# Mehran-Memon/fspann-query-system

Hardware: AMD Instinct MI355X
Metric: queries/sec @ recall@10, SIFT-1M-shaped synthetic data d=128 B=256 (higher is better)
Workload: dtype f64

## Files before the change

fspann-query-system_amd/csrc/route_lazy.hip.h:

```cpp
#pragma once
#include "route.hip.h"

namespace fspann {

constexpr uint64_t kLzEmpty = ~0ull;
constexpr int kLzThreads = 256;
constexpr int kLzEntriesMax = 1024;
constexpr int kLzCollMax = 256;
constexpr int lz_ht_size(int kEnt) { return 2 * kEnt; }
constexpr int lz_sort_max(int kEnt) { return kEnt - 128; }
constexpr size_t lz_order_bytes(int TP) {
    return static_cast<size_t>(TP + 2) * 8 + ((static_cast<size_t>(TP + 1) * 4 + 7) & ~size_t(7)) + static_cast<size_t>(TP) * 8 +
           ((static_cast<size_t>(TP) * 2 + 3) & ~size_t(3));
}
constexpr size_t lz_lds_bytes(int kEnt, int TD, int P) {
    const size_t tp = static_cast<size_t>(TD) * P, ord_gk = lz_order_bytes(TD * P), gk = static_cast<size_t>(lz_sort_max(kEnt)) * 4;
    return static_cast<size_t>(lz_ht_size(kEnt)) * 8 + tp * 16 + static_cast<size_t>(kEnt) * 4 + 4096 +
           (((ord_gk > gk ? ord_gk : gk) + 7) & ~size_t(7)) + static_cast<size_t>(TD) * 8 + static_cast<size_t>(kEnt) * 2 +
           static_cast<size_t>(lz_sort_max(kEnt)) * 2 * 2 + static_cast<size_t>(TD) * 4 +
           (kEnt != 512 ? static_cast<size_t>(TD) * 4 + tp * 4 : 0);
}
static_assert(lz_lds_bytes(512, 16, 5) == 20152 && lz_lds_bytes(512, 16, 5) + 256 <= 160 * 1024 / 8, "eight per CU at 16 x 5");
constexpr int lz_stage_u(int) { return 4; }
constexpr int lz_keep(int) { return 8; }

#ifdef FSPANN_DEBUG_STAMPS
__device__ __forceinline__ long long dbg_hw_where() {
    uint32_t hw, xcc;
    asm volatile("s_getreg_b32 %0, hwreg(HW_REG_HW_ID)" : "=s"(hw));
    asm volatile("s_getreg_b32 %0, hwreg(HW_REG_XCC_ID)" : "=s"(xcc));
    return (static_cast<long long>(xcc) << 32) | hw;
}
#endif

__device__ __forceinline__ int wave_cut1024(const int32_t* bins, int need, int lane, int* before) {
    const int4* b4 = reinterpret_cast<const int4*>(bins) + lane * 4;
    const int4 v0 = b4[0], v1 = b4[1], v2 = b4[2], v3 = b4[3];
    const int vals[16] = {v0.x, v0.y, v0.z, v0.w, v1.x, v1.y, v1.z, v1.w, v2.x, v2.y, v2.z, v2.w, v3.x, v3.y, v3.z, v3.w};
    int sum = 0;
#pragma unroll
    for (int i = 0; i < 16; i++) sum += vals[i];
    int incl = sum;
#pragma unroll
    for (int off = 1; off < 64; off <<= 1) {
        const int v = __shfl_up(incl, off);
        if (lane >= off) incl += v;
    }
    const int excl = incl - sum;
    const unsigned long long bm = __ballot((incl >= need) && (excl < need));
    if (bm == 0) {
        *before = __shfl(incl, 63) - __shfl(v3.w, 63);
        return 1023;
    }
    const int src = __ffsll(static_cast<long long>(bm)) - 1;
    int cum = excl, bb = 15;
    bool found = false;
#pragma unroll
    for (int i = 0; i < 16; i++) {
        if (!found) {
            if (cum + vals[i] >= need) { bb = i; found = true; }
            else cum += vals[i];
        }
    }
    *before = __shfl(cum, src);
    return __shfl(lane * 16 + bb, src);
}

template <int kThreads, int kEnt = kLzEntriesMax, bool kChk = true, int kTD = 0, int kP = 0, bool kList = false>
__device__ __forceinline__ void route_lazy_run(const RouteParams& prm, unsigned char* smem, const int64_t q_first, const int64_t q_stride, const int block_id) {
    int4* probe_in = prm.probe_g;
    int32_t* nprobe_in = prm.nprobe_g;
    int tid = threadIdx.x;
    constexpr int nthreads = kThreads;
    constexpr int nwv = kThreads / 64;
    int lane = tid & 63, wave = __builtin_amdgcn_readfirstlane(tid >> 6);
    const int TD = kTD > 0 ? kTD : prm.TD, P = kP > 0 ? kP : prm.P, S = (kTD > 0) ? 64 : prm.S;
    const int TP = TD * P;
    const int SP = (S + 63) >> 6;

    constexpr int kLzHtSize = lz_ht_size(kEnt), kLzEntries = kEnt, kLzSortMax = lz_sort_max(kEnt);
    constexpr int kLzStageU = lz_stage_u(kEnt), kLzKeep = lz_keep(kEnt);
    static_assert(kEnt == 512 || kEnt == 1024 || kEnt == 2048, "size classes");
    static_assert(!(kChk && kEnt == 512), "the 512-entry class has no registers for the check");
    size_t o = 0;
    uint64_t* ht = reinterpret_cast<uint64_t*>(smem + o);        o += static_cast<size_t>(kLzHtSize) * 8;
    int4* plist = reinterpret_cast<int4*>(smem + o);             o += static_cast<size_t>(TP) * 16;
    uint32_t* pre = reinterpret_cast<uint32_t*>(smem + o);       o += static_cast<size_t>(kEnt) * 4;
    int32_t* bins = reinterpret_cast<int32_t*>(smem + o);        o += 1024 * 4;
    const size_t o_ord = o;
    uint2* pkv = reinterpret_cast<uint2*>(smem + o);             o += (static_cast<size_t>(TP) + 2) * 8;
    int32_t* pcs = reinterpret_cast<int32_t*>(smem + o);         o += (static_cast<size_t>(TP) + 1) * 4;
    o = (o + 7) & ~size_t(7);
    int64_t* pbase = reinterpret_cast<int64_t*>(smem + o);       o += static_cast<size_t>(TP) * 8;
    uint16_t* ord = reinterpret_cast<uint16_t*>(smem + o);
    uint32_t* gk = reinterpret_cast<uint32_t*>(smem + o_ord);
    o = o_ord + ((max(lz_order_bytes(TP), static_cast<size_t>(kLzSortMax) * 4) + 7) & ~size_t(7));
    int64_t* ids_base = reinterpret_cast<int64_t*>(smem + o);    o += static_cast<size_t>(TD) * 8;
    uint16_t* ulist = reinterpret_cast<uint16_t*>(smem + o);     o += static_cast<size_t>(kLzEntries) * 2;
    uint16_t* rk = reinterpret_cast<uint16_t*>(smem + o);        o += static_cast<size_t>(kLzSortMax) * 2;
    uint16_t* lrank = reinterpret_cast<uint16_t*>(smem + o);     o += static_cast<size_t>(kLzSortMax) * 2;
    int32_t* nprobe_l = reinterpret_cast<int32_t*>(smem + o);    o += static_cast<size_t>(TD) * 4;
    int32_t* part0 = reinterpret_cast<int32_t*>(smem + o);       if (kEnt != 512) o += static_cast<size_t>(TD) * 4;
    int32_t* pglob = reinterpret_cast<int32_t*>(smem + o);
    int32_t* c_elem = bins;
    int32_t* c_lt = bins + kLzCollMax;
    int32_t* c_id = bins + 2 * kLzCollMax;
    int32_t* c_seq = bins + 3 * kLzCollMax;

    __shared__ int s_u, s_R, s_ncoll, s_bad, s_b, s_cnt, s_short, s_susp;
    constexpr uint32_t ht_mask = kLzHtSize - 1;
    constexpr int ht_shift = (kEnt == 2048) ? 32 - 12 : (kEnt == 1024) ? 32 - 11 : 32 - 10;
    unsigned long long lt_mask = 0;

    for (int i = tid; i < TD; i += nthreads) { ids_base[i] = prm.tables[i].ids_base; if (kChk) part0[i] = static_cast<int32_t>(prm.tables[i].part_base); }
    for (int i = tid; i < kLzHtSize; i += nthreads) ht[i] = kLzEmpty;
    if (kChk && prm.bin16) for (int i = tid; i < 1024; i += nthreads) bins[i] = 0;
    if (block_id == 0 && tid == 0) *prm.ovf_next = 0;
    __syncthreads();

    auto present = [&](int32_t id) -> bool {
        uint32_t slot = (static_cast<uint32_t>(id) * 2654435761u) >> ht_shift;
        const uint32_t stp = ((static_cast<uint32_t>(id) * 0x85EBCA6Bu) >> ht_shift) | 1u;
        for (int tries = 0; tries < kLzHtSize; tries++) {
            const uint64_t e = ht[slot];
            if (e == kLzEmpty) return false;
            if (static_cast<uint32_t>(e >> 32) == static_cast<uint32_t>(id)) return true;
            slot = (slot + stp) & ht_mask;
        }
        return false;
    };
    auto insert = [&](int32_t id, uint32_t low, uint32_t* slot_out) -> bool {
        const uint64_t mine = (static_cast<uint64_t>(static_cast<uint32_t>(id)) << 32) | low;
        uint32_t slot = (static_cast<uint32_t>(id) * 2654435761u) >> ht_shift;
        const uint32_t stp = ((static_cast<uint32_t>(id) * 0x85EBCA6Bu) >> ht_shift) | 1u;
        for (int tries = 0; tries < kLzHtSize; tries++) {
            const uint64_t old = atomicCAS(reinterpret_cast<unsigned long long*>(&ht[slot]), kLzEmpty, mine);
            if (old == kLzEmpty) { *slot_out = slot; return true; }
            if (static_cast<uint32_t>(old >> 32) == static_cast<uint32_t>(id)) {
                if (static_cast<uint32_t>(old) > low) atomicMin(reinterpret_cast<unsigned long long*>(&ht[slot]), mine);
                return false;
            }
            slot = (slot + stp) & ht_mask;
        }
        s_bad = 1;
        return false;
    };

#ifdef FSPANN_DEBUG_STAMPS
#define LZ_STAMP(i) do { if (prm.dbg && tid == 0 && qi == block_id) prm.dbg[block_id * 16 + (i)] = wall_clock64(); } while (0)
#else
#define LZ_STAMP(i) do { } while (0)
#endif
#ifdef FSPANN_LZ_STOP_AFTER
#define LZ_STOP(n) if (FSPANN_LZ_STOP_AFTER == (n) && prm.nq > 0) { __syncthreads(); if (tid == 0) prm.out_count[qi] = 0;               \
        const int used_ = min(s_u, kLzEntries); for (int i_ = tid; i_ < used_; i_ += nthreads) ht[ulist[i_]] = kLzEmpty; __syncthreads(); continue; }
#else
#define LZ_STOP(n)
#endif
#define LZ_FOR_TUPLES(RA, RB, BODY)                                                                                   \
    do {                                                                                                              \
        const int nit_ = ((RB) - (RA)) * SP;                                                                          \
        for (int it0_ = wave; it0_ < nit_; it0_ += nwv * kLzStageU) {                                                 \
            uint64_t entv_[kLzStageU];                                                                                \
            int scv_[kLzStageU];                                                                                      \
            _Pragma("unroll") for (int v_ = 0; v_ < kLzStageU; v_++) {                                                \
                const int it_ = it0_ + v_ * nwv;                                                                      \
                entv_[v_] = kLzEmpty; scv_[v_] = 0;                                                                   \
                if (it_ < nit_) {                                                                                     \
                    const int rr_ = (RA) + it_ / SP, pos_ = (it_ % SP) * 64 + lane;                                   \
                    const int pi_ = ord[rr_];                                                                         \
                    const int4 pr_ = plist[pi_];                                                                      \
                    scv_[v_] = pr_.y;                                                                                 \
                    if (pos_ < pr_.w) entv_[v_] = prm.ids_bk[pbase[pi_] + pos_];                                      \
                }                                                                                                     \
            }                                                                                                         \
            _Pragma("unroll") for (int v_ = 0; v_ < kLzStageU; v_++) {                                                \
                if (it0_ + v_ * nwv >= nit_) continue;                                                                \
                int32_t id = static_cast<int32_t>(entv_[v_] >> 32);                              \
                const uint32_t bf = static_cast<uint32_t>(entv_[v_]); (void)bf;                                       \
                const int sc = scv_[v_]; (void)sc;                                                                    \
                if (id >= 0 && prm.deleted_bits && ((prm.deleted_bits[id >> 5] >> (id & 31)) & 1u)) id = -1;  \
                BODY                                                                                                  \
            }                                                                                                         \
        }                                                                                                             \
    } while (0)
#define LZ_INSERT(COND, LOW)                                                                                          \
    do {                                                                                                              \
        bool created_ = false;                                                                                        \
        uint32_t slot_ = 0;                                                                                           \
        if (COND) created_ = insert(id, (LOW), &slot_);                                                               \
        const unsigned long long bm_ = __ballot(created_);                                                            \
        if (bm_) {                                                                                                    \
            int base_ = 0;                                                                                            \
            if (lane == 0) base_ = atomicAdd(&s_u, __popcll(bm_));                                                    \
            base_ = __shfl(base_, 0);                                                                                 \
            const int at_ = base_ + __popcll(bm_ & lt_mask);                                                          \
            if (created_ && at_ < kLzEntries) ulist[at_] = static_cast<uint16_t>(slot_);                              \
        }                                                                                                             \
    } while (0)

    const int64_t nq_eff = kList ? static_cast<int64_t>(*prm.qcount) : prm.nq;
    for (int64_t qs = q_first; qs < nq_eff; qs += q_stride) {
        const int64_t qi = kList ? static_cast<int64_t>(prm.qlist[qs]) : qs;
        LZ_STAMP(0);
        if (prm.probe_G > 0) {
            const int G = (kTD > 0) ? 16 : prm.probe_G, lgG = 31 - __clz(G), ngroups = nthreads >> lgG;
            const int grp_in_wave = lane >> lgG, gl = lane & (G - 1), grp = tid >> lgG;
            int32_t* w3 = reinterpret_cast<int32_t*>(pre) + grp * (2 * P - 1) * 3;
            for (int t0 = 0; t0 < TD; t0 += ngroups) {
                const int td = t0 + grp;
                const bool act = td < TD;
                const int tdc = act ? td : 0;
                const int Wc = (kTD > 0) ? 1 : prm.W;
#ifdef FSPANN_DEBUG_STAMPS
                long long* pst = (prm.dbg && tid == 0 && qi == block_id && t0 == 0) ? prm.dbg + (static_cast<long long>(gridDim.x) + block_id) * 16 : nullptr;
#else
                long long* pst = nullptr;
#endif
                const int np = route_probe_table<int4*, kP, (kTD > 0 ? 1 : 0)>(prm, act, prm.codes + (qi * TD + tdc) * Wc, prm.tables[tdc], G, gl, grp_in_wave,
                                                                             w3, plist + tdc * P, pst);
                if (act && gl == 0) nprobe_l[td] = np;
            }
            __syncthreads();
            for (int i = tid; i < TP; i += nthreads) {
                const int td = i / P, step = i - td * P;
                int4 e = make_int4(-1, 0x7FFF, 0, 0);
                if (step < nprobe_l[td]) e = plist[i];
                plist[i] = e;
                pbase[i] = ids_base[td] + e.z;
                if (kChk) pglob[i] = part0[td] + e.x;
                pkv[i] = make_uint2((static_cast<uint32_t>(e.y) << 16) | static_cast<uint32_t>(i), static_cast<uint32_t>(e.w));
            }
        } else {
            for (int i = tid; i < TP; i += nthreads) {
                const int td = i / P, step = i - td * P;
                int4 e = make_int4(-1, 0x7FFF, 0, 0);
                if (step < nprobe_in[qi * TD + td]) e = probe_in[qi * TP + i];
                plist[i] = e;
                pbase[i] = ids_base[td] + e.z;
                if (kChk) pglob[i] = part0[td] + e.x;
                pkv[i] = make_uint2((static_cast<uint32_t>(e.y) << 16) | static_cast<uint32_t>(i), static_cast<uint32_t>(e.w));
            }
        }
        if (tid == 0) {
            s_u = 0; s_R = TP; s_ncoll = 0; s_bad = 0; s_short = 0; s_susp = 0;
            if (TP & 1) pkv[TP] = make_uint2(0xFFFFFFFFu, 0u);
        }
        __syncthreads();
        LZ_STAMP(1);
        LZ_STOP(1)
        asm volatile("" : "+v"(tid));
        lane = tid & 63; wave = __builtin_amdgcn_readfirstlane(tid >> 6);
        lt_mask = (1ull << lane) - 1ull;
        constexpr int kChkU = 5;
        uint2 chk_v[kChkU];
        int chk_n[kChkU];
        const int chk_cps = prm.bin16_shift - 2;
        const int chk_items = (kChk && prm.bin16) ? (TP << chk_cps) : 0;
        const bool chk_once = chk_items <= nthreads * kChkU;
        auto chk_load = [&](const int it0) {
#pragma unroll
            for (int v = 0; v < kChkU; v++) {
                const int it = it0 + v * nthreads;
                chk_v[v] = make_uint2(0u, 0u); chk_n[v] = 0;
                if (it < chk_items) {
                    const int pi = it >> chk_cps, ch = it & ((1 << chk_cps) - 1);
                    const int4 pr = plist[pi];
                    const int rem = pr.w - ch * 4;
                    if (pr.x >= 0 && rem > 0) {
                        chk_v[v] = *reinterpret_cast<const uint2*>(prm.bin16 + (static_cast<int64_t>(pglob[pi]) << prm.bin16_shift) + ch * 4);
                        chk_n[v] = min(rem, 4);
                    }
                }
            }
        };
        auto chk_count = [&]() {
            bool sus = false;
#pragma unroll
            for (int v = 0; v < kChkU; v++) {
#pragma unroll
                for (int k = 0; k < 4; k++) {
                    if (k < chk_n[v]) {
                        const uint32_t b16 = ((k < 2 ? chk_v[v].x : chk_v[v].y) >> ((k & 1) * 16)) & 0xFFFFu;
                        const uint32_t sh = (b16 & 7u) * 4u;
                        const uint32_t old = atomicAdd(reinterpret_cast<uint32_t*>(bins) + ((b16 & 8191u) >> 3), 1u << sh);
                        sus = sus || (((old >> sh) & 15u) >= 8u);
                    }
                }
            }
            if (sus) s_susp = 1;
        };
        if (chk_items > 0 && chk_once) chk_load(tid);
        for (int i = tid; i < TP; i += nthreads) {
            const uint2 me = pkv[i];
            const uint32_t mk = me.x;
            int rank = 0, cum = 0;
            const uint4* kv4 = reinterpret_cast<const uint4*>(pkv);
#pragma unroll 4
            for (int j = 0; j < (TP + 1) / 2; j++) {
                const uint4 kv = kv4[j];
                const bool b0 = kv.x < mk, b1 = kv.z < mk;
                rank += b0 + b1;
                cum += (b0 ? kv.y : 0u) + (b1 ? kv.w : 0u);
            }
            ord[rank] = static_cast<uint16_t>(i);
            pcs[rank] = cum;
            if ((mk >> 16) == 0x7FFFu) atomicMin(&s_R, rank);
            if (rank == TP - 1) pcs[TP] = cum + static_cast<int>(me.y);
        }
        if (chk_items > 0) {
            if (chk_once) chk_count();
            else for (int it0 = tid; it0 < chk_items; it0 += nthreads * kChkU) { chk_load(it0); chk_count(); }
        }
        __syncthreads();
        LZ_STAMP(2);
        LZ_STOP(2)
        const int R = s_R;
        bool overflow = false;
        if (chk_items > 0 && s_susp) {
            uint32_t* mark = reinterpret_cast<uint32_t*>(ht);
            uint64_t* cl = ht + 128;
            uint64_t* cf = cl + 256;
            constexpr int kChkList = 256;
            static_assert(128 + 2 * 256 <= lz_ht_size(512), "the check's scratch fits the smallest hash table");
            for (int i = tid; i < 256; i += nthreads) mark[i] = 0u;
            for (int i = tid; i < 1024; i += nthreads) bins[i] = 0;
            __syncthreads();
            for (int it = tid; it < chk_items; it += nthreads) {
                const int pi = it >> chk_cps, ch = it & ((1 << chk_cps) - 1);
                const int4 pr = plist[pi];
                const int rem = pr.w - ch * 4;
                if (pr.x < 0 || rem <= 0) continue;
                const uint2 vv = *reinterpret_cast<const uint2*>(prm.bin16 + (static_cast<int64_t>(pglob[pi]) << prm.bin16_shift) + ch * 4);
                for (int k = 0; k < min(rem, 4); k++) {
                    const uint32_t b16 = ((k < 2 ? vv.x : vv.y) >> ((k & 1) * 16)) & 0xFFFFu, f = b16 & 8191u;
                    const uint32_t sh = (f & 7u) * 4u;
                    const uint32_t old = atomicAdd(reinterpret_cast<uint32_t*>(bins) + (f >> 3), 1u << sh);
                    if (((old >> sh) & 15u) >= 8u) atomicOr(&mark[f >> 5], 1u << (f & 31u));
                }
            }
            __syncthreads();
            for (int it = tid; it < chk_items; it += nthreads) {
                const int pi = it >> chk_cps, ch = it & ((1 << chk_cps) - 1);
                const int4 pr = plist[pi];
                const int rem = pr.w - ch * 4;
                if (pr.x < 0 || rem <= 0) continue;
                const uint2 vv = *reinterpret_cast<const uint2*>(prm.bin16 + (static_cast<int64_t>(pglob[pi]) << prm.bin16_shift) + ch * 4);
                for (int k = 0; k < min(rem, 4); k++) {
                    const uint32_t b16 = ((k < 2 ? vv.x : vv.y) >> ((k & 1) * 16)) & 0xFFFFu, f = b16 & 8191u;
                    if (!((mark[f >> 5] >> (f & 31u)) & 1u)) continue;
                    const int32_t id = prm.ids[pbase[pi] + ch * 4 + k];
                    if (prm.deleted_bits && ((prm.deleted_bits[id >> 5] >> (id & 31)) & 1u)) continue;
                    const int c = atomicAdd(&s_ncoll, 1);
                    if (c < kChkList) cl[c] = (static_cast<uint64_t>(b16) << 32) | static_cast<uint32_t>(id);
                }
            }
            __syncthreads();
            const int ncl = s_ncoll;
            if (ncl > kChkList) {
                overflow = true;
            } else {
                for (int i = tid; i < ncl; i += nthreads) {
                    const uint64_t me = cl[i];
                    bool first = true;
                    for (int j = 0; j < i; j++) first = first && (cl[j] != me);
                    cf[i] = first ? me : ~0ull;
                }
                __syncthreads();
                for (int i = tid; i < ncl; i += nthreads) {
                    const uint64_t me = cf[i];
                    if (me == ~0ull) continue;
                    int same = 0;
                    for (int j = 0; j < ncl; j++) same += (cf[j] != ~0ull) && ((cf[j] >> 32) == (me >> 32));
                    if (same >= 9) s_bad = 1;
                }
            }
            __syncthreads();
            if (s_bad) overflow = true;
            for (int i = tid; i < 128 + 2 * kChkList; i += nthreads) ht[i] = kLzEmpty;
            if (tid == 0) s_ncoll = 0;
            __syncthreads();
        }
        int r0 = 0, u = 0;
        int dbg_outer = 0, dbg_inner = 0, dbg_reload = 0, dbg_nitb = 0;
        (void)dbg_outer; (void)dbg_inner; (void)dbg_reload; (void)dbg_nitb;
        bool force_full = false;
        while (r0 < R && u < prm.limit && !overflow) {
            const int need = prm.limit - u;
            int r_fit = r0, r_nofit = R;
            for (int c0 = r0 + 1; c0 <= R; c0 += 64) {
                const int r = c0 + lane;
                const bool bnd = (r <= R) && (r == R || (pkv[ord[r]].x >> 16) != (pkv[ord[r - 1]].x >> 16));
                const unsigned long long bb = __ballot(bnd);
                const unsigned long long bf = __ballot(bnd && (pcs[r] - pcs[r0] <= need));
                if (bf) r_fit = c0 + 63 - __clzll(static_cast<long long>(bf));
                if (bb & ~bf) { r_nofit = c0 + __ffsll(static_cast<long long>(bb & ~bf)) - 1; break; }
            }
            const int rb0 = r_fit, rb1 = (r_fit < R) ? r_nofit : R;
            const int npB = rb1 - rb0;
            auto tuples_per_id = [](const int tuples, const int ids) -> int {
                return (tuples >= 8 * ids) ? 128 : (tuples >= 4 * ids) ? 64 : (tuples >= 3 * ids) ? 48 : (tuples >= 2 * ids) ? 32 : (2 * tuples >= 3 * ids) ? 24 : 16;
            };
            int boost = 16;
            if (r0 > 0 && u > 0) boost = min(64, tuples_per_id(pcs[r0], u));
            int L = 64;
            if (npB > 0 && SP == 1 && !force_full) {
                const int tuplesB = max(pcs[rb1] - pcs[rb0], 1);
                const int want = (2 * 64 * ((need * boost) >> 4)) / tuplesB + 8;
                L = (want <= 8) ? 8 : (want <= 16) ? 16 : (want <= 32) ? 32 : 64;
            }
            const int Lsh = 31 - __clz(L);
            const int G = 64 >> Lsh;
            const int nitB = (L == 64) ? npB * SP : (npB + G - 1) / G;
            const bool keep = (nitB > 0) && (nitB <= nwv * kLzKeep);
            dbg_outer++; dbg_reload += (nitB > 0 && !keep); dbg_nitb = max(dbg_nitb, nitB);
            int32_t idr[kLzKeep];
            uint32_t bfr[kLzKeep];
            if (keep) {
#pragma unroll
                for (int k = 0; k < kLzKeep; k++) {
                    const int it = wave + k * nwv;
                    idr[k] = -1; bfr[k] = 0;
                    if (it < nitB) {
                        int pidx, pos;
                        if (L == 64) { pidx = it / SP; pos = (it % SP) * 64 + lane; }
                        else { pidx = it * G + (lane >> Lsh); pos = lane & (L - 1); }
                        if (pidx < npB) {
                            const int pi = ord[rb0 + pidx];
                            const int4 pr = plist[pi];
                            if (pos < pr.w) {
                                const uint64_t ent = prm.ids_bk[pbase[pi] + pos];
                                idr[k] = static_cast<int32_t>(ent >> 32);
                                bfr[k] = static_cast<uint32_t>(ent) | ((L < 64 && pos == L - 1 && pr.w > L) ? 0x80000000u : 0u);
                            }
                        }
                    }
                }
            }
            for (int i = tid; i < 1024; i += nthreads) bins[i] = 0;
            if (r_fit > r0) {
                LZ_FOR_TUPLES(r0, r_fit, {
                    LZ_INSERT(id >= 0, (static_cast<uint32_t>(sc) << kBucketBits) | bf);
                });
            }
            __syncthreads();
            LZ_STAMP(8);
            u = s_u;
            if (s_bad) { overflow = true; break; }
            if (u >= prm.limit || rb0 >= R) {
                r0 = rb0;
                __syncthreads();
                continue;
            }
            const uint32_t sc_hi = (pkv[ord[rb0]].x >> 16) << kBucketBits;
            if (keep) {
#pragma unroll
                for (int k = 0; k < kLzKeep; k++) {
                    int32_t id = idr[k];
                    if (id >= 0 && prm.deleted_bits && ((prm.deleted_bits[id >> 5] >> (id & 31)) & 1u)) id = -1;
                    if (id >= 0) {
                        if (present(id)) id = -1;
                        else atomicAdd(&bins[(bfr[k] & 0xFFFFFu) >> (kBucketBits - 10)], 1);
                    }
                    idr[k] = id;
                }
            } else {
                LZ_FOR_TUPLES(rb0, rb1, {
                    if (id >= 0 && !present(id)) atomicAdd(&bins[bf >> (kBucketBits - 10)], 1);
                });
            }
            __syncthreads();
            LZ_STAMP(10);
            int lo = 0;
            bool redo_full = false;
            if (rb0 > 0 && u > 0) boost = min(64, tuples_per_id(pcs[rb0], u));
            while (true) {
                const int missing = prm.limit - u;
                const int ask = max(missing, min((missing * boost) >> 4, ((prm.lazy_cap - u) * 3) >> 2));
                if (wave == 0) {
                    int before = 0;
                    const int b = (lo == 0) ? wave_cut1024(bins, ask, lane, &before)
                                            : lo + wave_find_cut(bins + lo, 1024 - lo, ask, lane, &before);
                    if (lane == 0) { s_b = b; s_cnt = before + bins[b]; }
                }
                __syncthreads();
                LZ_STAMP(11);
                dbg_inner++;
                const int b = s_b;
                const int offered = s_cnt;
                if (u + offered > prm.lazy_cap) { overflow = true; break; }
                if (keep && L < 64) {
                    bool shortp = false;
#pragma unroll
                    for (int k = 0; k < kLzKeep; k++)
                        shortp = shortp || ((bfr[k] & 0x80000000u) && static_cast<int>((bfr[k] & 0xFFFFFu) >> (kBucketBits - 10)) <= b);
                    if (__any(shortp) && lane == 0) s_short = 1;
                    __syncthreads();
                    if (s_short) { redo_full = true; break; }
                }
                if (keep) {
                    int total = 0;
#pragma unroll
                    for (int k = 0; k < kLzKeep; k++) {
                        const int bin = static_cast<int>((bfr[k] & 0xFFFFFu) >> (kBucketBits - 10));
                        if (idr[k] >= 0 && bin >= lo && bin <= b) {
                            uint32_t slot = 0;
                            const bool c = insert(idr[k], sc_hi | (bfr[k] & 0xFFFFFu), &slot);
                            idr[k] = c ? -2 : -1;
                            if (c) bfr[k] = slot;
                        }
                        total += __popcll(__ballot(idr[k] == -2));
                    }
                    if (total) {
                        int base = 0;
                        if (lane == 0) base = atomicAdd(&s_u, total);
                        base = __shfl(base, 0);
#pragma unroll
                        for (int k = 0; k < kLzKeep; k++) {
                            const bool c = (idr[k] == -2);
                            const unsigned long long bm = __ballot(c);
                            const int at = base + __popcll(bm & lt_mask);
                            if (c && at < kLzEntries) ulist[at] = static_cast<uint16_t>(bfr[k]);
                            if (c) idr[k] = -1;
                            base += __popcll(bm);
                        }
                    }
                } else {
                    LZ_FOR_TUPLES(rb0, rb1, {
                        const int bin = static_cast<int>(bf >> (kBucketBits - 10));
                        LZ_INSERT(id >= 0 && bin >= lo && bin <= b, sc_hi | bf);
                    });
                }
                __syncthreads();
                LZ_STAMP(12);
                const int u_was = u;
                u = s_u;
                if (s_bad) { overflow = true; break; }
                if (u >= prm.limit || b >= 1023) break;
                boost = tuples_per_id(offered, max(u - u_was, 1));
                lo = b + 1;
                __syncthreads();
            }
            if (overflow) break;
            if (redo_full) {
                r0 = rb0;
                force_full = true;
                __syncthreads();
                if (tid == 0) s_short = 0;
                __syncthreads();
                continue;
            }
            force_full = false;
            r0 = rb1;
            __syncthreads();
        }
        LZ_STAMP(3);
        LZ_STOP(3)
        const int nsel = u;
        if (nsel > kLzSortMax) overflow = true;
        if (!overflow) {
            const int nout = min(nsel, prm.limit);
            const uint32_t smin = pkv[ord[0]].x >> 16;
            auto coarse = [&](const uint32_t key) -> uint32_t { return min((key - (smin << kBucketBits)) >> (kBucketBits - 6), 1023u); };
            for (int i = tid; i < kEnt; i += nthreads) pre[i] = (i < nsel) ? static_cast<uint32_t>(ht[ulist[i]]) : 0xFFFFFFFFu;
            for (int i = tid; i < kLzSortMax / 2; i += nthreads) reinterpret_cast<uint32_t*>(rk)[i] = 0u;
            for (int i = tid; i < 1024; i += nthreads) bins[i] = 0;
            __syncthreads();
            LZ_STAMP(4);
            for (int i = tid; i < nsel; i += nthreads) atomicAdd(&bins[coarse(pre[i])], 1);
            __syncthreads();
            if (wave == 0) {
                int4* b4 = reinterpret_cast<int4*>(bins) + lane * 4;
                int4 v[4] = {b4[0], b4[1], b4[2], b4[3]};
                int* vals = reinterpret_cast<int*>(v);
                int sum = 0;
#pragma unroll
                for (int i = 0; i < 16; i++) { const int t = vals[i]; vals[i] = sum; sum += t; }
                int incl = sum;
#pragma unroll
                for (int off = 1; off < 64; off <<= 1) {
                    const int t = __shfl_up(incl, off);
                    if (lane >= off) incl += t;
                }
                const int excl = incl - sum;
#pragma unroll
                for (int i = 0; i < 16; i++) vals[i] += excl;
                b4[0] = v[0]; b4[1] = v[1]; b4[2] = v[2]; b4[3] = v[3];
            }
            __syncthreads();
            for (int i = tid; i < nsel; i += nthreads) {
                const uint32_t my = pre[i];
                gk[atomicAdd(&bins[coarse(my)], 1)] = my;
            }
            __syncthreads();
            for (int i = tid; i < nsel; i += nthreads) {
                const uint32_t my = pre[i];
                const uint32_t c = coarse(my);
                const int g1 = bins[c], g0 = c ? bins[c - 1] : 0;
                int lt = g0;
                for (int j = g0; j < g1; j++) lt += gk[j] < my;
                atomicAdd(reinterpret_cast<uint32_t*>(rk) + (lt >> 1), 1u << ((lt & 1) * 16));
                lrank[i] = static_cast<uint16_t>(lt);
            }
            __syncthreads();
            for (int i = tid; i < nsel; i += nthreads) {
                const int lt = lrank[i];
                if (rk[lt] != 1) {
                    if (rk[lt] >= 9) s_bad = 1;
                    const int c = atomicAdd(&s_ncoll, 1);
                    if (c < kLzCollMax) { c_elem[c] = i; c_lt[c] = lt; c_id[c] = static_cast<int32_t>(ht[ulist[i]] >> 32); c_seq[c] = 0x7FFFFFFF; }
                }
            }
            __syncthreads();
            LZ_STAMP(5);
            LZ_STOP(5)
            const int ncoll = s_ncoll;
#ifdef FSPANN_DEBUG_STAMPS
            if (tid == 0 && prm.dbg && qi == block_id) { prm.dbg[block_id * 16 + 13] = ncoll; prm.dbg[block_id * 16 + 15] = nsel; prm.dbg[block_id * 16 + 14] = dbg_outer | (dbg_inner << 8) | (dbg_reload << 16) | (static_cast<long long>(dbg_nitb) << 24); }
#endif
            if (ncoll > kLzCollMax || s_bad) {
                overflow = true;
            } else {
                if (ncoll > 0) {
                    const int npair = ncoll * TD;
                    for (int t0 = tid; t0 < npair; t0 += nthreads * 4) {
                        int32_t idxv[4];
#pragma unroll
                        for (int v = 0; v < 4; v++) {
                            const int t = t0 + v * nthreads;
                            idxv[v] = (t < npair) ? prm.inv[static_cast<int64_t>(t % TD) * prm.n_ids + c_id[t / TD]] : -1;
                        }
#pragma unroll
                        for (int v = 0; v < 4; v++) {
                            const int t = t0 + v * nthreads;
                            const int32_t idx = idxv[v];
                            if (idx < 0) continue;
                            const int c = t / TD, td = t - c * TD;
                            for (int step = 0; step < P; step++) {
                                const int4 e = plist[td * P + step];
                                if (e.x >= 0 && idx >= e.z && idx < e.z + e.w) { atomicMin(&c_seq[c], (td * P + step) * S + (idx - e.z)); break; }
                            }
                        }
                    }
                    for (int c = tid; c < ncoll; c += nthreads) c_elem[c] = static_cast<int32_t>(pre[c_elem[c]]);
                    __syncthreads();
                    for (int c = tid; c < ncoll; c += nthreads) {
                        const int32_t my = c_elem[c];
                        const int myseq = c_seq[c];
                        int rank = c_lt[c];
#pragma unroll 4
                        for (int c2 = 0; c2 < ncoll; c2++) rank += (c_elem[c2] == my) && (c_seq[c2] < myseq);
                        if (rank < nout) {
                            prm.out_ids[qi * prm.out_cap + rank] = c_id[c];
                            if (prm.out_score) prm.out_score[qi * prm.out_cap + rank] = static_cast<int32_t>(static_cast<uint32_t>(my) >> kBucketBits);
                        }
                    }
                }
                for (int i = tid; i < nsel; i += nthreads) {
                    const int lt = lrank[i];
                    if (lt < nout && rk[lt] == 1) {
                        const uint64_t e = ht[ulist[i]];
                        prm.out_ids[qi * prm.out_cap + lt] = static_cast<int32_t>(e >> 32);
                        if (prm.out_score) prm.out_score[qi * prm.out_cap + lt] = static_cast<int32_t>(static_cast<uint32_t>(e) >> kBucketBits);
                    }
                }
            }
            if (!overflow && tid == 0) prm.out_count[qi] = nout;
        }
        if (overflow) {
            if (prm.probe_G > 0) {
                for (int i = tid; i < TP; i += nthreads) probe_in[qi * TP + i] = plist[i];
                for (int i = tid; i < TD; i += nthreads) nprobe_in[qi * TD + i] = nprobe_l[i];
            }
            if (tid == 0) {
                prm.out_count[qi] = kRoutePending;
                prm.ovf_list[atomicAdd(prm.ovf_count, 1)] = static_cast<int32_t>(qi);
            }
        }
        if (qs + q_stride >= nq_eff) {
            LZ_STAMP(6);
            LZ_STAMP(7);
            break;
        }
        __syncthreads();
        LZ_STAMP(6);
        const int used = min(s_u, kLzEntries);
        for (int i = tid; i < used; i += nthreads) ht[ulist[i]] = kLzEmpty;
        if (kChk && prm.bin16) for (int i = tid; i < 1024; i += nthreads) bins[i] = 0;
        __syncthreads();
        LZ_STAMP(7);
    }
#undef LZ_STOP
#undef LZ_STAMP
#undef LZ_FOR_TUPLES
#undef LZ_INSERT
}

template <int kThreads, int kEnt, bool kChk, int kTD = 0, int kP = 0>
__global__ __launch_bounds__(kThreads, (kEnt <= 512 ? (kTD > 0 ? 8 : 6) : (kEnt <= 1024 ? 4 : 2))) void route_select_lazy_kernel(RouteParams prm) {
    extern __shared__ __align__(16) unsigned char smem[];
#ifdef FSPANN_DEBUG_STAMPS
    if (prm.dbg && threadIdx.x == 0) prm.dbg[blockIdx.x * 16 + 9] = dbg_hw_where();
#endif
    route_lazy_run<kThreads, kEnt, kChk, kTD, kP>(prm, smem, static_cast<int64_t>(blockIdx.x), static_cast<int64_t>(gridDim.x), static_cast<int>(blockIdx.x));
}

template <int kThreads, int kEnt, bool kChk>
__global__ __launch_bounds__(kThreads, (kEnt <= 512 ? 6 : (kEnt <= 1024 ? 4 : 2))) void route_select_lazy_list_kernel(RouteParams prm) {
    extern __shared__ __align__(16) unsigned char smem[];
    if (static_cast<int64_t>(blockIdx.x) >= static_cast<int64_t>(*prm.qcount)) {
        if (blockIdx.x == 0 && threadIdx.x == 0) *prm.ovf_next = 0;
        return;
    }
    route_lazy_run<kThreads, kEnt, kChk, 0, 0, true>(prm, smem, static_cast<int64_t>(blockIdx.x), static_cast<int64_t>(gridDim.x), static_cast<int>(blockIdx.x));
}

}
```

Before: 27.15 million.

## Keep sort keys in registers and fuse rank, collision and output passes

The final rank/select stage now keeps each thread's keys and ids in registers instead of staging them through a shared `pre` array. The separate rk/lrank tie-count arrays and their passes are gone: equal-key counts are computed during the bucket scan, and unique elements write their output directly. The bin clearing moves into the preceding loop, several __syncthreads are removed, and two barriers become a raw lgkmcnt wait plus s_barrier. This cuts LDS traffic and block barriers per query, at the cost of more register pressure and a hand-written barrier that assumes no pending global stores need ordering.

```diff
diff --git a/fspann-query-system_amd/csrc/route_lazy.hip.h b/fspann-query-system_amd/csrc/route_lazy.hip.h
--- a/fspann-query-system_amd/csrc/route_lazy.hip.h
+++ b/fspann-query-system_amd/csrc/route_lazy.hip.h
@@ -33,6 +33,8 @@
 }
 #endif
 
+__device__ __forceinline__ void lz_lds_barrier() { asm volatile("s_waitcnt lgkmcnt(0)\n\ts_barrier" ::: "memory"); }
+
 __device__ __forceinline__ int wave_cut1024(const int32_t* bins, int need, int lane, int* before) {
     const int4* b4 = reinterpret_cast<const int4*>(bins) + lane * 4;
     const int4 v0 = b4[0], v1 = b4[1], v2 = b4[2], v3 = b4[3];
@@ -85,7 +87,7 @@
     size_t o = 0;
     uint64_t* ht = reinterpret_cast<uint64_t*>(smem + o);        o += static_cast<size_t>(kLzHtSize) * 8;
     int4* plist = reinterpret_cast<int4*>(smem + o);             o += static_cast<size_t>(TP) * 16;
-    uint32_t* pre = reinterpret_cast<uint32_t*>(smem + o);       o += static_cast<size_t>(kEnt) * 4;
+    uint32_t* wscr = reinterpret_cast<uint32_t*>(smem + o);      o += static_cast<size_t>(kEnt) * 4;
     int32_t* bins = reinterpret_cast<int32_t*>(smem + o);        o += 1024 * 4;
     const size_t o_ord = o;
     uint2* pkv = reinterpret_cast<uint2*>(smem + o);             o += (static_cast<size_t>(TP) + 2) * 8;
@@ -97,15 +99,16 @@
     o = o_ord + ((max(lz_order_bytes(TP), static_cast<size_t>(kLzSortMax) * 4) + 7) & ~size_t(7));
     int64_t* ids_base = reinterpret_cast<int64_t*>(smem + o);    o += static_cast<size_t>(TD) * 8;
     uint16_t* ulist = reinterpret_cast<uint16_t*>(smem + o);     o += static_cast<size_t>(kLzEntries) * 2;
-    uint16_t* rk = reinterpret_cast<uint16_t*>(smem + o);        o += static_cast<size_t>(kLzSortMax) * 2;
-    uint16_t* lrank = reinterpret_cast<uint16_t*>(smem + o);     o += static_cast<size_t>(kLzSortMax) * 2;
+    unsigned char* cscr = smem + o;                              o += static_cast<size_t>(kLzSortMax) * 2 * 2;
     int32_t* nprobe_l = reinterpret_cast<int32_t*>(smem + o);    o += static_cast<size_t>(TD) * 4;
     int32_t* part0 = reinterpret_cast<int32_t*>(smem + o);       if (kEnt != 512) o += static_cast<size_t>(TD) * 4;
     int32_t* pglob = reinterpret_cast<int32_t*>(smem + o);
-    int32_t* c_elem = bins;
-    int32_t* c_lt = bins + kLzCollMax;
-    int32_t* c_id = bins + 2 * kLzCollMax;
-    int32_t* c_seq = bins + 3 * kLzCollMax;
+    uint32_t* c_key = wscr;
+    int32_t* c_id = reinterpret_cast<int32_t*>(wscr) + kLzCollMax;
+    int32_t* c_seq = reinterpret_cast<int32_t*>(cscr);
+    uint16_t* c_lt = reinterpret_cast<uint16_t*>(cscr + static_cast<size_t>(kLzCollMax) * 4);
+    static_assert(static_cast<size_t>(kEnt) * 4 >= static_cast<size_t>(kLzCollMax) * 8 && static_cast<size_t>(kLzSortMax) * 4 >= static_cast<size_t>(kLzCollMax) * 6 &&
+                  kLzSortMax < 65536, "the collision records fit their bytes");
 
     __shared__ int s_u, s_R, s_ncoll, s_bad, s_b, s_cnt, s_short, s_susp;
     constexpr uint32_t ht_mask = kLzHtSize - 1;
@@ -206,7 +209,7 @@
         if (prm.probe_G > 0) {
             const int G = (kTD > 0) ? 16 : prm.probe_G, lgG = 31 - __clz(G), ngroups = nthreads >> lgG;
             const int grp_in_wave = lane >> lgG, gl = lane & (G - 1), grp = tid >> lgG;
-            int32_t* w3 = reinterpret_cast<int32_t*>(pre) + grp * (2 * P - 1) * 3;
+            int32_t* w3 = reinterpret_cast<int32_t*>(wscr) + grp * (2 * P - 1) * 3;
             for (int t0 = 0; t0 < TD; t0 += ngroups) {
                 const int td = t0 + grp;
                 const bool act = td < TD;
@@ -552,6 +555,7 @@
             }
             force_full = false;
             r0 = rb1;
+            if (r0 >= R || u >= prm.limit) for (int i = tid; i < 1024; i += nthreads) bins[i] = 0;
             __syncthreads();
         }
         LZ_STAMP(3);
@@ -560,15 +564,24 @@
         if (nsel > kLzSortMax) overflow = true;
         if (!overflow) {
             const int nout = min(nsel, prm.limit);
+            constexpr int kPer = (kLzSortMax + nthreads - 1) / nthreads;
             const uint32_t smin = pkv[ord[0]].x >> 16;
             auto coarse = [&](const uint32_t key) -> uint32_t { return min((key - (smin << kBucketBits)) >> (kBucketBits - 6), 1023u); };
-            for (int i = tid; i < kEnt; i += nthreads) pre[i] = (i < nsel) ? static_cast<uint32_t>(ht[ulist[i]]) : 0xFFFFFFFFu;
-            for (int i = tid; i < kLzSortMax / 2; i += nthreads) reinterpret_cast<uint32_t*>(rk)[i] = 0u;
-            for (int i = tid; i < 1024; i += nthreads) bins[i] = 0;
+            uint32_t keyr[kPer];
+            int32_t idk[kPer];
+#pragma unroll
+            for (int k = 0; k < kPer; k++) {
+                keyr[k] = 0xFFFFFFFFu; idk[k] = -1;
+                if (k * nthreads + wave * 64 >= nsel) continue;
+                const int i = tid + k * nthreads;
+                if (i < nsel) {
+                    const uint64_t e = ht[ulist[i]];
+                    keyr[k] = static_cast<uint32_t>(e); idk[k] = static_cast<int32_t>(e >> 32);
+                    atomicAdd(&bins[coarse(keyr[k])], 1);
+                }
+            }
             __syncthreads();
             LZ_STAMP(4);
-            for (int i = tid; i < nsel; i += nthreads) atomicAdd(&bins[coarse(pre[i])], 1);
-            __syncthreads();
             if (wave == 0) {
                 int4* b4 = reinterpret_cast<int4*>(bins) + lane * 4;
                 int4 v[4] = {b4[0], b4[1], b4[2], b4[3]};
@@ -588,30 +601,33 @@
                 b4[0] = v[0]; b4[1] = v[1]; b4[2] = v[2]; b4[3] = v[3];
             }
             __syncthreads();
-            for (int i = tid; i < nsel; i += nthreads) {
-                const uint32_t my = pre[i];
-                gk[atomicAdd(&bins[coarse(my)], 1)] = my;
-            }
-            __syncthreads();
-            for (int i = tid; i < nsel; i += nthreads) {
-                const uint32_t my = pre[i];
+#pragma unroll
+            for (int k = 0; k < kPer; k++) {
+                if (k * nthreads + wave * 64 >= nsel) continue;
+                if (tid + k * nthreads < nsel) gk[atomicAdd(&bins[coarse(keyr[k])], 1)] = keyr[k];
+            }
+            __syncthreads();
+#pragma unroll
+            for (int k = 0; k < kPer; k++) {
+                if (k * nthreads + wave * 64 >= nsel) continue;
+                if (tid + k * nthreads >= nsel) continue;
+                const uint32_t my = keyr[k];
                 const uint32_t c = coarse(my);
                 const int g1 = bins[c], g0 = c ? bins[c - 1] : 0;
-                int lt = g0;
-                for (int j = g0; j < g1; j++) lt += gk[j] < my;
-                atomicAdd(reinterpret_cast<uint32_t*>(rk) + (lt >> 1), 1u << ((lt & 1) * 16));
-                lrank[i] = static_cast<uint16_t>(lt);
-            }
-            __syncthreads();
-            for (int i = tid; i < nsel; i += nthreads) {
-                const int lt = lrank[i];
-                if (rk[lt] != 1) {
-                    if (rk[lt] >= 9) s_bad = 1;
-                    const int c = atomicAdd(&s_ncoll, 1);
-                    if (c < kLzCollMax) { c_elem[c] = i; c_lt[c] = lt; c_id[c] = static_cast<int32_t>(ht[ulist[i]] >> 32); c_seq[c] = 0x7FFFFFFF; }
-                }
-            }
-            __syncthreads();
+                int lt = g0, eq = 0;
+                for (int j = g0; j < g1; j++) { const uint32_t g = gk[j]; lt += g < my; eq += g == my; }
+                if (eq == 1) {
+                    if (lt < nout) {
+                        prm.out_ids[qi * prm.out_cap + lt] = idk[k];
+                        if (prm.out_score) prm.out_score[qi * prm.out_cap + lt] = static_cast<int32_t>(my >> kBucketBits);
+                    }
+                } else {
+                    if (eq >= 9) s_bad = 1;
+                    const int cc = atomicAdd(&s_ncoll, 1);
+                    if (cc < kLzCollMax) { c_key[cc] = my; c_lt[cc] = static_cast<uint16_t>(lt); c_id[cc] = idk[k]; c_seq[cc] = 0x7FFFFFFF; }
+                }
+            }
+            lz_lds_barrier();
             LZ_STAMP(5);
             LZ_STOP(5)
             const int ncoll = s_ncoll;
@@ -620,48 +636,37 @@
 #endif
             if (ncoll > kLzCollMax || s_bad) {
                 overflow = true;
-            } else {
-                if (ncoll > 0) {
-                    const int npair = ncoll * TD;
-                    for (int t0 = tid; t0 < npair; t0 += nthreads * 4) {
-                        int32_t idxv[4];
-#pragma unroll
-                        for (int v = 0; v < 4; v++) {
-                            const int t = t0 + v * nthreads;
-                            idxv[v] = (t < npair) ? prm.inv[static_cast<int64_t>(t % TD) * prm.n_ids + c_id[t / TD]] : -1;
+            } else if (ncoll > 0) {
+                const int npair = ncoll * TD;
+                for (int t0 = tid; t0 < npair; t0 += nthreads * 4) {
+                    int32_t idxv[4];
+#pragma unroll
+                    for (int v = 0; v < 4; v++) {
+                        const int t = t0 + v * nthreads;
+                        idxv[v] = (t < npair) ? prm.inv[static_cast<int64_t>(t % TD) * prm.n_ids + c_id[t / TD]] : -1;
+                    }
+#pragma unroll
+                    for (int v = 0; v < 4; v++) {
+                        const int t = t0 + v * nthreads;
+                        const int32_t idx = idxv[v];
+                        if (idx < 0) continue;
+                        const int c = t / TD, td = t - c * TD;
+                        for (int step = 0; step < P; step++) {
+                            const int4 e = plist[td * P + step];
+                            if (e.x >= 0 && idx >= e.z && idx < e.z + e.w) { atomicMin(&c_seq[c], (td * P + step) * S + (idx - e.z)); break; }
                         }
-#pragma unroll
-                        for (int v = 0; v < 4; v++) {
-                            const int t = t0 + v * nthreads;
-                            const int32_t idx = idxv[v];
-                            if (idx < 0) continue;
-                            const int c = t / TD, td = t - c * TD;
-                            for (int step = 0; step < P; step++) {
-                                const int4 e = plist[td * P + step];
-                                if (e.x >= 0 && idx >= e.z && idx < e.z + e.w) { atomicMin(&c_seq[c], (td * P + step) * S + (idx - e.z)); break; }
-                            }
-                        }
-                    }
-                    for (int c = tid; c < ncoll; c += nthreads) c_elem[c] = static_cast<int32_t>(pre[c_elem[c]]);
-                    __syncthreads();
-                    for (int c = tid; c < ncoll; c += nthreads) {
-                        const int32_t my = c_elem[c];
-                        const int myseq = c_seq[c];
-                        int rank = c_lt[c];
+                    }
+                }
+                lz_lds_barrier();
+                for (int c = tid; c < ncoll; c += nthreads) {
+                    const uint32_t my = c_key[c];
+                    const int myseq = c_seq[c];
+                    int rank = c_lt[c];
 #pragma unroll 4
-                        for (int c2 = 0; c2 < ncoll; c2++) rank += (c_elem[c2] == my) && (c_seq[c2] < myseq);
-                        if (rank < nout) {
-                            prm.out_ids[qi * prm.out_cap + rank] = c_id[c];
-                            if (prm.out_score) prm.out_score[qi * prm.out_cap + rank] = static_cast<int32_t>(static_cast<uint32_t>(my) >> kBucketBits);
-                        }
-                    }
-                }
-                for (int i = tid; i < nsel; i += nthreads) {
-                    const int lt = lrank[i];
-                    if (lt < nout && rk[lt] == 1) {
-                        const uint64_t e = ht[ulist[i]];
-                        prm.out_ids[qi * prm.out_cap + lt] = static_cast<int32_t>(e >> 32);
-                        if (prm.out_score) prm.out_score[qi * prm.out_cap + lt] = static_cast<int32_t>(static_cast<uint32_t>(e) >> kBucketBits);
+                    for (int c2 = 0; c2 < ncoll; c2++) rank += (c_key[c2] == my) && (c_seq[c2] < myseq);
+                    if (rank < nout) {
+                        prm.out_ids[qi * prm.out_cap + rank] = c_id[c];
+                        if (prm.out_score) prm.out_score[qi * prm.out_cap + rank] = static_cast<int32_t>(my >> kBucketBits);
                     }
                 }
             }
```

Result: no change. 27.11 million (-0.2%).
